# graehl/carmel

Hardware: AMD Instinct MI355X
Metric: arc-updates/sec (EM iterations/sec x derivation-lattice arcs swept per iteration) (higher is better)
Workload: dtype f64; 1 GPU; c4: synthetic 1000000-state / 9999990-arc WFST, 1000000 training pairs per GPU (random walks of 5-40 arcs), conditional normalisation, cached lattices; parallelism=corpus-sharded x1, none

## Files before the change

carmel_amd/csrc/engine.cpp:

```cpp
#include <hip/hip_runtime.h>
#include <chrono>
#include <cmath>
#include <cstdio>
#include <cstring>
#include <cstdlib>
#include <limits>
#include <string>
#include <thread>
#include <unordered_map>
#include <vector>
#include "engine.hpp"
#include "options.hpp"
#include "host/refhash.hpp"
#include "rng.hpp"
#include "unrolled_args.hpp"

int unrolled_try_build(carmel_hip_trainer* t, int host_threads, uint8_t* has_derivation, carmel_hip_lattice_stats* stats);
int gpu_build_lattices(carmel_hip_trainer* t, const BuildOptions& opt, uint8_t* has_derivation, carmel_hip_lattice_stats* stats,
                       bool& done);
int gpu_tables_for_host_layout(carmel_hip_trainer* t, const std::vector<uint32_t>& lane_arc, const std::vector<uint32_t>& wave_arc);
int carmel_hip_debug_lattice_fingerprint_impl(carmel_hip_trainer* t, uint64_t* out);
int build_run_tables(carmel_hip_trainer* t);
int exchange_weights_in(carmel_hip_trainer* t, ExchangePlan* xp, const TransArgs& T, bool need_x);
int exchange_counts_out(carmel_hip_trainer* t, ExchangePlan* xp, const TransArgs& T);
// ... 176 lines not shown
    int arc = weights_ahead_drop(t);
    if (arc) return arc;
  }
  layout_changed(t);
  if (t->scalars_pending) {
    (void)hipStreamSynchronize(t->side);
    t->scalars_pending = false;
  }
  t->build_prune = prune;
  t->build_threads = host_threads;
  if (t->matrix) {
    HIPCHK(hipStreamSynchronize(t->stream));
    matrix_release(t->matrix);
    t->matrix = nullptr;
  }
  {
    int rc = unrolled_try_build(t, host_threads, has_derivation, stats);
    if (rc) return rc;
    if (t->unrolled) return CARMEL_HIP_OK;
  }
  auto t0 = std::chrono::steady_clock::now();
  BuildOptions opt;
  opt.prune = prune != 0;
  opt.threads = host_threads;
  if (const char* e = lib_opt("lane_states")) opt.lane_states = (uint32_t)atoi(e);
  if (const char* e = lib_opt("tile_sweep")) opt.tile_sweep = atoi(e) != 0;
  if (const char* e = lib_opt("lane_fused")) opt.lane_fused = atoi(e) != 0;
  if (lib_opt("transpose") && atoi(lib_opt("transpose")) == 0) opt.lane_fused = false;
  if (const char* e = lib_opt("lane_chunks")) opt.lane_chunks = (uint32_t)std::max(1, atoi(e));
  if (const char* e = lib_opt("lane_window")) opt.lane_window = (uint32_t)std::max(0, atoi(e));
  if (const char* e = lib_opt("lane_window_min")) opt.lane_window_min = (uint32_t)std::max(0, atoi(e));
  if (const char* e = lib_opt("wave_ring")) opt.wave_ring = atoi(e) != 0;
  if (const char* e = lib_opt("wave_min_width")) opt.wave_min_width = opt.wave_lane_min_width = atof(e);
  {
    const bool want_gpu = !(lib_opt("gpu_build") && atoi(lib_opt("gpu_build")) == 0) &&
                          !(lib_opt("transpose") && atoi(lib_opt("transpose")) == 0);
    bool probe_ok = true;
    if (want_gpu && t->corpus.n_pairs > 4096) {
      const uint64_t np = t->corpus.n_pairs, n_probe = 64;
      for (uint64_t k = 0; k < n_probe && probe_ok; ++k) {
        const uint64_t p = k * (np / n_probe);
        PairLattice pl;
        bool hd = false;
        build_pair_lattice(t->w, t->corpus.in_sym.data() + t->corpus.in_off[p], (uint32_t)(t->corpus.in_off[p + 1] - t->corpus.in_off[p]),
                           t->corpus.out_sym.data() + t->corpus.out_off[p], (uint32_t)(t->corpus.out_off[p + 1] - t->corpus.out_off[p]),
                           opt.prune, pl, hd);
        if (pl.explored_states > 200 || (hd && (pl.n_states > opt.lane_states || pl.edges.size() > 200))) opt.gpu_large_caps = true;
        if (pl.explored_states > 1024 || (hd && (pl.cyclic || pl.n_states > 1023 || pl.edges.size() > 1536))) probe_ok = false;
      }
    }
    if (want_gpu && probe_ok) {
      bool done = false;
      int rc = gpu_build_lattices(t, opt, has_derivation, stats, done);
      if (rc) return rc;
      if (!done && !opt.gpu_large_caps) {
        opt.gpu_large_caps = true;
        rc = gpu_build_lattices(t, opt, has_derivation, stats, done);
        if (rc) return rc;
        if (!done) opt.gpu_large_caps = false;
      }
      if (done) {
        if (lib_opt("timing")) fprintf(stderr, "timing: lattices built on the GPU\n");
        rc = build_run_tables(t);
        if (stats) stats->device_bytes = t->device_bytes;
        return rc;
      }
// ... 1473 lines not shown
```

carmel_amd/csrc/host_api.cpp:

```cpp
#include <cstdlib>
#include <algorithm>
#include <cstring>
#include <string>
#include "../../include/carmel_hip.h"
#include "options.hpp"
#include "lattice.hpp"

using namespace carmel_hip;

struct carmel_hip_host_lattices {
  HostWfst w;
  HostCorpus c;
  LatticeSet L;
  std::string err;
};

extern "C" {

int carmel_hip_host_build(carmel_hip_host_lattices** out, uint32_t n_states, uint32_t final_state, uint64_t n_arcs,
                          const uint32_t* src, const uint32_t* dst, const uint32_t* in_sym, const uint32_t* out_sym,
                          uint64_t n_pairs, const uint64_t* in_off, const uint32_t* cin, const uint64_t* out_off,
                          const uint32_t* cout, const double* pair_weight, int prune, int threads,
                          uint32_t small_pairs, uint32_t small_states, int lane_states) {
  if (!out) return CARMEL_HIP_ERR_ARG;
  carmel_hip_host_lattices* h = new carmel_hip_host_lattices();
  h->w.n_states = n_states;
  h->w.final_state = final_state;
  h->w.n_arcs = n_arcs;
  h->w.src.assign(src, src + n_arcs);
  h->w.dst.assign(dst, dst + n_arcs);
  h->w.in.assign(in_sym, in_sym + n_arcs);
  h->w.out.assign(out_sym, out_sym + n_arcs);
  h->w.build_index();
  h->c.n_pairs = n_pairs;
  h->c.in_off.assign(in_off, in_off + n_pairs + 1);
  h->c.out_off.assign(out_off, out_off + n_pairs + 1);
  h->c.in_sym.assign(cin, cin + in_off[n_pairs]);
  h->c.out_sym.assign(cout, cout + out_off[n_pairs]);
  if (pair_weight)
    h->c.weight.assign(pair_weight, pair_weight + n_pairs);
  else
    h->c.weight.assign(n_pairs, 1.0);
  BuildOptions opt;
  opt.prune = prune != 0;
  opt.threads = threads;
  if (small_pairs) opt.small_pairs = small_pairs;
  if (small_states) opt.small_states = small_states;
  if (lane_states >= 0) opt.lane_states = (uint32_t)lane_states;
  if (const char* e = lib_opt("lane_window")) opt.lane_window = (uint32_t)std::max(0, atoi(e));
  if (const char* e = lib_opt("tile_sweep")) opt.tile_sweep = atoi(e) != 0;
  if (const char* e = lib_opt("lane_fused")) opt.lane_fused = atoi(e) != 0;
  if (const char* e = lib_opt("lane_window_min")) opt.lane_window_min = (uint32_t)std::max(0, atoi(e));
  if (lane_states == 0 && !lib_opt("wave_min_width")) opt.wave = false;
  if (const char* e = lib_opt("wave_ring")) opt.wave_ring = atoi(e) != 0;
  if (const char* e = lib_opt("wave_min_width")) opt.wave_min_width = opt.wave_lane_min_width = atof(e);
  if (!build_lattices(h->w, h->c, opt, h->L, h->err)) {
    delete h;
    return CARMEL_HIP_ERR_ARG;
  }
  *out = h;
  return CARMEL_HIP_OK;
}

void carmel_hip_host_dims(carmel_hip_host_lattices* h, uint64_t* dims) {
  dims[0] = h->L.bundles.size();
  dims[1] = h->L.in_off.size();
  dims[2] = h->L.in_arcs.size();
  dims[3] = h->L.level_off.size();
  dims[4] = h->L.pair_id.size();
  dims[5] = h->L.classes.size();
  dims[6] = h->L.n_kept;
  dims[7] = h->L.n_cyclic;
  dims[8] = h->L.explored_states;
  dims[9] = h->L.explored_arcs;
  dims[10] = h->L.lane_groups.size();
  dims[11] = h->L.lane_fwd.size();
  dims[12] = h->L.lane_pair.size();
  dims[13] = h->L.lane_classes.size();
  dims[14] = h->L.total_states;
  dims[15] = h->L.total_arcs;
  dims[16] = h->L.last_pre_states;
  dims[17] = h->L.last_post_states;
  dims[18] = h->L.last_post_arcs;
}

// ... 105 lines not shown
```

carmel_amd/csrc/lattice.cpp:

```cpp
#include "lattice.hpp"
#include "options.hpp"
#include <algorithm>
#include <functional>
#include <chrono>
#include <cmath>
#include <cstring>
#include <limits>
#include <numeric>
#include <thread>
#include <atomic>

namespace carmel_hip {
void build_transpose(LatticeSet& out, uint64_t n_arcs, int nt);


void HostWfst::build_index() {
  idx_off.assign((size_t)n_states + 1, 0);
  for (uint64_t k = 0; k < n_arcs; ++k) idx_off[src[k] + 1]++;
  for (uint32_t s = 0; s < n_states; ++s) idx_off[s + 1] += idx_off[s];
  idx_key.resize(n_arcs);
  idx_arc.resize(n_arcs);
  std::vector<uint64_t> cur(idx_off.begin(), idx_off.end() - 1);
  for (uint64_t k = 0; k < n_arcs; ++k) {
    uint64_t p = cur[src[k]]++;
// ... 504 lines not shown
                        bool prune, PairLattice& lat, bool& has_deriv) {
  Scratch sc;
  build_pair_lattice_impl(w, in, n_in, out, n_out, prune, lat, has_deriv, sc);
}

namespace {

struct BundlePlan {
  std::vector<uint32_t> pairs;
  uint64_t n_states = 0, n_arcs = 0;
  uint32_t n_levels = 0;
  bool cyclic = false;
};

}

bool build_lattices(const HostWfst& w, const HostCorpus& c, const BuildOptions& opt, LatticeSet& out,
                    std::string& err) {
  if (w.idx_off.size() != (size_t)w.n_states + 1) {
    err = "WFST index not built";
    return false;
  }
  const uint64_t np = c.n_pairs;
  const bool timing = lib_opt("timing") != nullptr;
  auto tick = std::chrono::steady_clock::now();
  auto phase = [&](const char* name) {
    if (!timing) return;
    auto now = std::chrono::steady_clock::now();
    fprintf(stderr, "timing: lattice build: %-28s %8.3f s\n", name, std::chrono::duration<double>(now - tick).count());
    tick = now;
  };
  std::vector<PairLattice> lats(np);
  out = LatticeSet();
  out.has_deriv.assign(np, 0);
  int nt = opt.threads > 0 ? opt.threads : std::min(32, (int)std::thread::hardware_concurrency());
  if (nt < 1) nt = 1;
  if ((uint64_t)nt > np) nt = (int)std::max<uint64_t>(1, np);
  {
    std::atomic<uint64_t> next(0);
    const uint64_t batch = std::max<uint64_t>(1, std::min<uint64_t>(256, np / ((uint64_t)nt * 8)));
    auto work = [&]() {
      Scratch sc;
      for (;;) {
        uint64_t p0 = next.fetch_add(batch);
        if (p0 >= np) break;
        uint64_t p1 = std::min(np, p0 + batch);
        for (uint64_t p = p0; p < p1; ++p) {
          bool hd = false;
          build_pair_lattice_impl(w, c.in_sym.data() + c.in_off[p], (uint32_t)(c.in_off[p + 1] - c.in_off[p]),
                                  c.out_sym.data() + c.out_off[p], (uint32_t)(c.out_off[p + 1] - c.out_off[p]),
                                  opt.prune, lats[p], hd, sc);
          out.has_deriv[p] = hd;
          PairLattice& L = lats[p];
          if (hd && !L.cyclic && opt.lane_window && L.n_states > opt.lane_window_min && L.n_states <= LANE_STATE_MASK) {
            std::vector<uint32_t>& cnt = sc.span_cnt;
            std::vector<uint32_t>& nid = sc.span_id;
            cnt.assign((size_t)L.n_levels + 2, 0);
            for (uint32_t st = 0; st < L.n_states; ++st) cnt[L.level[st] + 1]++;
            for (size_t k = 1; k < cnt.size(); ++k) cnt[k] += cnt[k - 1];
            nid.resize(L.n_states);
            for (uint32_t st = 0; st < L.n_states; ++st) nid[st] = cnt[L.level[st]]++;
            uint32_t sp = 1;
            for (auto& e : L.edges) sp = std::max(sp, nid[e.dst] - nid[e.src]);
            L.span = sp;
          }
        }
// ... 667 lines not shown
    for (uint64_t a = 0; a < w.n_arcs; ++a) cnt[a + 1] += cnt[a];
    const uint64_t total = cnt[w.n_arcs];
    out.arc_off = cnt;
    out.slot_pos.resize(total);
    in_threads([&](int t) {
      const uint64_t lo = arc_lo(t), hi = arc_lo(t + 1);
      for (uint64_t k = 0; k < nlane_rec; ++k) {
        const uint2_t r = out.lane_bwd[k];
        if ((r.x & LANE_VALID) && r.y >= lo && r.y < hi) out.slot_pos[cnt[r.y]++] = k;
      }
      for (uint64_t k = 0; k < nwave; ++k) {
        const uint32_t a = out.wave_bwd_arc[k];
        if (a != 0xffffffffu && a >= lo && a < hi) out.slot_pos[cnt[a]++] = out.wave_slot_base + k;
      }
      for (uint64_t k = 0; k < out.out_arcs.size(); ++k) {
        const uint32_t a = out.out_arcs[k].y;
        if (a >= lo && a < hi) out.slot_pos[cnt[a]++] = nlane + k;
      }
    });
    for (uint64_t a = 0; a < w.n_arcs; ++a)
      if (out.arc_off[a + 1] - out.arc_off[a] > 64)
        for (uint64_t j = out.arc_off[a]; j < out.arc_off[a + 1]; j += 4096) {
          out.hot_chunks.push_back(a);
          out.hot_chunks.push_back(j);
          out.hot_chunks.push_back(std::min(out.arc_off[a + 1], j + 4096));
        }
  }
  phase("slots by arc (counting sort)");
  build_transpose(out, w.n_arcs, nt);
  phase("transposition tables");
  return true;
}

void build_transpose(LatticeSet& out, uint64_t n_arcs, int nt) {
  const uint64_t N = out.slot_pos.size();
  out.t_buckets.clear();
  out.t_split_arcs.clear();
  if (N >= (1ull << 32) || N == 0) return;
  const uint64_t BK = out.bucket;
  {
    uint64_t a = 0;
    while (a < n_arcs) {
      uint64_t c = out.arc_off[a + 1] - out.arc_off[a];
      if (c > TRANS_HEAVY) {
        const bool split = c > BK;
        if (split) out.t_split_arcs.push_back((uint32_t)a);
        for (uint64_t g = out.arc_off[a]; g < out.arc_off[a + 1]; g += BK)
          out.t_buckets.push_back(TransBucket{g, (uint32_t)std::min<uint64_t>(BK, out.arc_off[a + 1] - g),
                                              (uint32_t)a, 1u, TRANS_SINGLE | (split ? TRANS_SPLIT : 0u)});
        ++a;
        continue;
      }
      uint64_t e = a, items = 0;
      while (e < n_arcs && e - a < BK) {
        uint64_t ce = out.arc_off[e + 1] - out.arc_off[e];
        if (ce > TRANS_HEAVY || items + ce > BK) break;
        items += ce;
        ++e;
      }
      out.t_buckets.push_back(TransBucket{out.arc_off[a], (uint32_t)items, (uint32_t)a, (uint32_t)(e - a), 0u});
      a = e;
    }
  }
  out.t_a_off.assign(n_arcs, 0);
  for (const TransBucket& B : out.t_buckets)
    if (!(B.flags & TRANS_SINGLE))
      for (uint32_t a = 0; a < B.n_arcs; ++a) out.t_a_off[B.arc_lo + a] = (uint16_t)(out.arc_off[B.arc_lo + a] - B.item_base);
  out.t_b_arc.assign(N, 0);
  out.t_b_rank.assign(N, 0);
  out.t_b_src.assign(N, 0);
  out.t_t_pos.assign(N, 0);
  out.t_t_src.assign(N, 0);
  const uint64_t tile_sz = out.tile;
  const uint64_t n_tiles = (out.n_post + tile_sz - 1) / tile_sz;
  out.t_tile_base.assign(n_tiles + 1, 0);
  std::vector<uint64_t> pos_of(N);
  {
    std::atomic<size_t> next(0);
    auto work = [&]() {
      std::vector<std::pair<uint64_t, uint32_t>> items;
      for (;;) {
        size_t b = next.fetch_add(16);
        if (b >= out.t_buckets.size()) break;
        size_t be = std::min(out.t_buckets.size(), b + 16);
        for (; b < be; ++b) {
          const TransBucket& B = out.t_buckets[b];
          items.resize(B.n_items);
          for (uint32_t r = 0; r < B.n_items; ++r) items[r] = {out.slot_pos[B.item_base + r], r};
          std::sort(items.begin(), items.end());
          uint64_t a = B.arc_lo;
          std::vector<uint16_t> arc_of_rank(B.n_items);
          if (B.flags & TRANS_SINGLE) {
            std::fill(arc_of_rank.begin(), arc_of_rank.end(), (uint16_t)0);
          } else {
// ... 57 lines not shown
```

carmel_amd/csrc/lattice.hpp:

```cpp
#pragma once
#include <cstdint>
#include <vector>
#include <string>

namespace carmel_hip {

struct HostWfst {
  uint32_t n_states = 0, final_state = 0;
  uint64_t n_arcs = 0;
  std::vector<uint32_t> src, dst, in, out, group;
  std::vector<uint64_t> idx_off;
  std::vector<uint64_t> idx_key;
  std::vector<uint32_t> idx_arc;
  void build_index();
};

struct HostCorpus {
  uint64_t n_pairs = 0;
  std::vector<uint64_t> in_off, out_off;
  std::vector<uint32_t> in_sym, out_sym;
  std::vector<double> weight;
};

struct PairLattice {
// ... 24 lines not shown
};
static_assert(sizeof(BundleDesc) == 64, "BundleDesc layout");

struct uint2_t {
  uint32_t x, y;
};

static const uint32_t LANE_CHUNK = 4;
static const uint32_t LANE_LAST = 0x80000000u;
static const uint32_t LANE_VALID = 0x40000000u;
static const uint32_t LANE_STATE_MASK = 0x3ffu;
static const uint32_t LANE_POS_SHIFT = 10;
static const uint32_t LANE_POS_MAX = (1u << 20) - 1;
#ifndef TRANS_K
#define TRANS_K 16
#endif
#ifndef TRANS_KT
#define TRANS_KT TRANS_K
#endif
#ifndef TRANS_KB
#define TRANS_KB TRANS_K
#endif
static const uint32_t TRANS_TILE = TRANS_KT * 1024, TRANS_BUCKET = TRANS_KB * 1024, TRANS_HEAVY = 2048, TRANS_SPLIT = 1u, TRANS_SINGLE = 2u;
static const uint32_t TILE_SWEEP_TILE = 8192, TILE_SWEEP_ALPHA_ROWS = 126, TILE_SWEEP_ROWS = 48, TILE_SWEEP_GROUPS = 16;
static const uint32_t TILE_SWEEP_LDS = TILE_SWEEP_TILE * 12 + TILE_SWEEP_ALPHA_ROWS * 64 * 8;
#ifndef LANE_FUSED_ROWS_N
#define LANE_FUSED_ROWS_N 16
#endif
static const uint32_t LANE_FUSED_ROWS = LANE_FUSED_ROWS_N, LANE_FUSED_TILE = LANE_FUSED_ROWS * 64;
struct TransBucket {
  uint64_t item_base;
  uint32_t n_items, arc_lo, n_arcs, flags;
};
struct LaneGroup {
  uint64_t stream_base;
  uint32_t maxlen;
  uint32_t n_lanes;
  uint32_t pair_base;
  uint32_t max_states;
  uint32_t window;
  uint32_t spill_row;
};
static_assert(sizeof(LaneGroup) == 32, "LaneGroup layout");

static const uint32_t WAVE_VALID = 0x80000000u;
static const uint32_t WAVE_MAX_STATES = 16384, WAVE_MAX_WIDTH = 1024;
static const uint32_t WAVE_RING_MAX = 1024, WAVE_RING_WIDTH = 64;
struct WaveDesc {
  uint64_t fwd_base;
  uint64_t bwd_base;
  uint32_t n_states, n_levels;
  uint32_t level_base;
  uint32_t pair;
  uint32_t max_width;
  uint32_t ring;
  double logw;
  uint64_t n_arcs;
  uint64_t spill_base;
};
static_assert(sizeof(WaveDesc) == 64, "WaveDesc layout");

struct LatticeSet {
  std::vector<WaveDesc> waves;
  std::vector<uint2_t> wave_fwd;
  std::vector<uint32_t> wave_bwd;
  std::vector<uint32_t> wave_bwd_arc;
// ... 9 lines not shown
  uint64_t wave_slot_base = 0;
  uint64_t wave_states = 0, wave_arcs = 0;
  std::vector<BundleDesc> bundles;
  std::vector<uint2_t> in_arcs, out_arcs;
  std::vector<uint32_t> in_off, out_off;
  std::vector<uint32_t> level_off;
  std::vector<uint32_t> pair_start, pair_final, pair_id;
  std::vector<double> pair_logw;
  struct LaunchClass {
    uint32_t first, count;
    uint32_t block;
    uint32_t max_states;
    bool serial;
  };
  std::vector<LaunchClass> classes;
  std::vector<LaneGroup> lane_groups;
  std::vector<uint2_t> lane_fwd, lane_bwd;
  std::vector<uint32_t> lane_pair, lane_nstates;
  std::vector<double> lane_logw;
  struct LaneClass {
    uint32_t first, count, max_states;
    uint32_t tile_first = 0, tile_count = 0;
    bool windowed = false;
  };
  uint64_t lane_spill_rows = 0;
  std::vector<LaneClass> lane_classes;
  bool lane_tiles_aligned = false;
  uint32_t tile = TRANS_TILE;
  bool tile_sweep = false;
  bool wave_gather = false;
  bool tables_deferred = false;
  bool lane_fused = false;
  uint32_t bucket = TRANS_BUCKET;
  std::vector<uint32_t> tile_group;
  uint64_t lane_states = 0, lane_arcs = 0;
  std::vector<uint32_t> state_orig;
  std::vector<uint64_t> arc_off;
  std::vector<uint64_t> slot_pos;
  std::vector<uint64_t> hot_chunks;
  uint64_t n_post = 0;
  std::vector<TransBucket> t_buckets;
  std::vector<uint64_t> t_tile_base;
  std::vector<uint16_t> t_b_arc;
  std::vector<uint16_t> t_b_rank;
  std::vector<uint32_t> t_b_src;
  std::vector<uint16_t> t_t_pos;
  std::vector<uint32_t> t_t_src;
  std::vector<uint16_t> t_a_off;
  std::vector<uint32_t> t_split_arcs;
  uint64_t total_states = 0, total_arcs = 0, max_levels = 0, n_cyclic = 0;
  uint64_t explored_states = 0, explored_arcs = 0;
  uint64_t last_pre_states = 0, last_post_states = 0, last_post_arcs = 0;
  std::vector<uint8_t> has_deriv;
  uint64_t n_kept = 0;
};

struct BuildOptions {
  bool prune = true;
  int threads = 0;
  uint32_t small_pairs = 64;
  uint32_t small_states = 2048;
  uint32_t lds_states_max = 16384;
  uint32_t lane_states = 96;
  uint32_t lane_window = 64;
  uint32_t lane_window_min = 40;
  bool keep_state_ids = false;
  bool gpu_large_caps = false;
  bool wave_ring = true;
  bool wave = true;
  double wave_min_width = 4.0;
  double wave_lane_min_width = 16.0;
  uint64_t wave_lane_threshold = 262144;
  uint32_t wave_lane_arcs = 2048;
  bool tile_sweep = true;
  bool wave_gather = false;
  bool device_tables = false;
  bool lane_fused = true;
  uint32_t lane_chunks = 1;
};

bool build_lattices(const HostWfst& w, const HostCorpus& c, const BuildOptions& opt, LatticeSet& out, std::string& err);

uint64_t assign_lane_classes(LatticeSet& out, const BuildOptions& opt, bool only_lanes);

void build_pair_lattice(const HostWfst& w, const uint32_t* in, uint32_t n_in, const uint32_t* out, uint32_t n_out,
                        bool prune, PairLattice& lat, bool& has_deriv);

}
```

carmel_amd/csrc/lattice_gpu.hip:

```cpp
#include <hip/hip_runtime.h>
#include <hipcub/hipcub.hpp>
#include <algorithm>
#include <chrono>
#include <functional>
#include <cmath>
#include <cstring>
#include <limits>
#include <vector>
#include "engine.hpp"
#include "options.hpp"

namespace {

struct GCaps {
  uint32_t cx, ce, ck, ch, threads;
};
const GCaps G_SMALL = {256, 448, 256, 512, 131072};
const GCaps G_LARGE = {1024, 2560, 1536, 2048, 65536};

enum { PF_HAS = 1, PF_FALLBACK = 2 };

struct GArgs {
  const uint64_t* idx_off;
  const uint64_t* idx_key;
// ... 507 lines not shown
  const uint32_t* rb = rec_bwd + (size_t)p * GK;
  const uint32_t* ra = rec_arc + (size_t)p * GK;
  for (uint32_t k = 0; k < e; ++k) {
    const uint32_t x = rf[k];
    const uint32_t bp = ((x >> LANE_POS_SHIFT) & LANE_POS_MAX) + shift;
    f[(size_t)k * 64] = (x & ~(LANE_POS_MAX << LANE_POS_SHIFT)) | (bp << LANE_POS_SHIFT);
    b[(size_t)(shift + k) * 64] = rb[k];
    items[it + k] = ((unsigned long long)ra[k] << 32) | (unsigned long long)(g.stream_base + (uint64_t)(shift + k) * 64 + lane);
  }
}

__global__ void slots_kernel(const unsigned long long* items, uint64_t n, uint64_t n_arcs, uint64_t* slot_pos, uint64_t* arc_off) {
  const uint64_t i = (uint64_t)blockIdx.x * blockDim.x + threadIdx.x;
  if (i >= n) return;
  const uint32_t a = (uint32_t)(items[i] >> 32);
  slot_pos[i] = items[i] & 0xffffffffull;
  const uint32_t prev = i ? (uint32_t)(items[i - 1] >> 32) : 0u;
  for (uint64_t x = (i ? (uint64_t)prev + 1 : 0); x <= a; ++x) arc_off[x] = i;
  if (i + 1 == n)
    for (uint64_t x = (uint64_t)a + 1; x <= n_arcs; ++x) arc_off[x] = n;
}

__global__ void bucket_end_kernel(const uint64_t* arc_off, uint64_t n_arcs, uint32_t* b_end, uint32_t BK ) {
  const uint64_t a = (uint64_t)blockIdx.x * blockDim.x + threadIdx.x;
  if (a >= n_arcs) return;
  const uint64_t limit = arc_off[a] + BK;
  uint64_t lo = a, hi = min(n_arcs, a + (uint64_t)BK);
  while (lo < hi) {
    const uint64_t m = (lo + hi + 1) >> 1;
    if (arc_off[m] <= limit) lo = m; else hi = m - 1;
  }
  b_end[a] = (uint32_t)lo;
}
__global__ void heavy_list_kernel(const uint64_t* arc_off, uint64_t n_arcs, uint32_t* list, uint32_t cap, uint32_t* n) {
  const uint64_t a = (uint64_t)blockIdx.x * blockDim.x + threadIdx.x;
  if (a >= n_arcs || arc_off[a + 1] - arc_off[a] <= TRANS_HEAVY) return;
  const uint32_t k = atomicAdd(n, 1u);
  if (k < cap) list[k] = (uint32_t)a;
}
__global__ void bucket_chain_kernel(const uint64_t* arc_off, const uint32_t* b_end, uint64_t n_arcs, const uint32_t* heavy,
                                    uint32_t n_heavy, TransBucket* buckets, uint32_t* split_arcs, uint32_t cap,
                                    uint32_t* n_out , uint32_t BK ) {
  if (blockIdx.x || threadIdx.x) return;
  uint64_t a = 0;
  uint32_t nb = 0, ns = 0, hp = 0;
  bool over = false;
  while (a < n_arcs) {
    const uint64_t c = arc_off[a + 1] - arc_off[a];
    if (c > TRANS_HEAVY) {
      const bool split = c > BK;
      if (split) {
        if (ns < cap) split_arcs[ns] = (uint32_t)a;
        ++ns;
      }
      for (uint64_t g = arc_off[a]; g < arc_off[a + 1]; g += BK) {
        if (nb < cap)
          buckets[nb] = TransBucket{g, (uint32_t)min((uint64_t)BK, arc_off[a + 1] - g), (uint32_t)a, 1u,
                                    TRANS_SINGLE | (split ? TRANS_SPLIT : 0u)};
        else
          over = true;
        ++nb;
      }
      ++a;
      continue;
    }
    uint64_t e = b_end[a];
    while (hp < n_heavy && heavy[hp] < a) ++hp;
    if (hp < n_heavy && heavy[hp] < e) e = heavy[hp];
    if (e == a) e = a + 1;
    if (nb < cap)
      buckets[nb] = TransBucket{arc_off[a], (uint32_t)(arc_off[e] - arc_off[a]), (uint32_t)a, (uint32_t)(e - a), 0u};
// ... 295 lines not shown
  fp(3, t->lane_pair.p, t->lane_pair.bytes());
  fp(4, t->lane_nstates.p, t->lane_nstates.bytes());
  fp(5, t->lane_logw.p, t->lane_logw.bytes());
  fp(6, t->t_buckets.p, t->t_buckets.bytes());
  fp(7, t->t_tile_base.p, t->t_tile_base.bytes());
  fp(8, t->t_b_arc.p, t->t_b_arc.bytes() & ~(size_t)3);
  fp(9, t->t_b_rank.p, t->t_b_rank.bytes() & ~(size_t)3);
  fp(10, t->t_b_src.p, t->t_b_src.bytes());
  fp(11, t->t_t_pos.p, t->t_t_pos.bytes() & ~(size_t)3);
  fp(12, t->t_t_src.p, t->t_t_src.bytes());
  fp(13, t->t_a_off.p, t->t_a_off.bytes() & ~(size_t)3);
  fp(14, t->t_split_arcs.p, t->t_split_arcs.bytes());
  fp(15, t->pair_w.p, t->pair_w.bytes());
  HIPCHK(hipGetLastError());
  HIPCHK(hipMemcpyAsync(out, acc.p, 16 * 8, hipMemcpyDeviceToHost, s));
  HIPCHK(hipStreamSynchronize(s));
  return CARMEL_HIP_OK;
}

static int gpu_tables_from_items(carmel_hip_trainer* t, DevBuf<char>& tmp, DevBuf<unsigned long long>& items, DevBuf<unsigned long long>& items_sorted,
                                 uint64_t n_items, uint64_t n_sort, uint64_t n_post, const std::function<void(const char*)>& lap) {
  const HostWfst& w = t->w;
  const LatticeSet& L = t->lat;
  hipStream_t s = t->stream;
  HIPCHK(sort_keys(tmp, items.p, items_sorted.p, n_sort, 32 + bits_for(w.n_arcs + 1), s));
  HIPCHK(t->arc_off.alloc(w.n_arcs + 1));
  HIPCHK(t->slot_pos.alloc(n_items));
  hipLaunchKernelGGL(slots_kernel, dim3((unsigned)((n_items + 255) / 256)), dim3(256), 0, s, items_sorted.p, n_items, w.n_arcs,
                     t->slot_pos.p, t->arc_off.p);
  t->hot_chunks.release();
  lap("slots by arc");
  DevBuf<uint32_t> b_end, d_nout;
  HIPCHK(b_end.alloc(w.n_arcs));
  HIPCHK(d_nout.alloc(4));
  hipLaunchKernelGGL(bucket_end_kernel, dim3((unsigned)((w.n_arcs + 255) / 256)), dim3(256), 0, s, t->arc_off.p, w.n_arcs, b_end.p, L.bucket);
  const uint32_t cap = (uint32_t)(2 * (n_items / L.bucket) + w.n_arcs / L.bucket + 2 * (n_items / TRANS_HEAVY) + 16);
  HIPCHK(t->t_buckets.alloc(cap));
  HIPCHK(t->t_split_arcs.alloc(cap));
  DevBuf<uint32_t> heavy, heavy_sorted;
  HIPCHK(heavy.alloc(cap));
  HIPCHK(heavy_sorted.alloc(cap));
  HIPCHK(hipMemsetAsync(d_nout.p, 0, 16, s));
  hipLaunchKernelGGL(heavy_list_kernel, dim3((unsigned)((w.n_arcs + 255) / 256)), dim3(256), 0, s, t->arc_off.p, w.n_arcs, heavy.p, cap,
                     d_nout.p + 3);
  uint32_t n_heavy = 0;
  HIPCHK(hipMemcpyAsync(&n_heavy, d_nout.p + 3, 4, hipMemcpyDeviceToHost, s));
  HIPCHK(hipStreamSynchronize(s));
  if (n_heavy > cap) return fail(CARMEL_HIP_ERR_HIP, "gpu lattice build: heavy-arc list overflow");
  if (n_heavy) HIPCHK(sort_keys(tmp, heavy.p, heavy_sorted.p, n_heavy, 32, s));
  hipLaunchKernelGGL(bucket_chain_kernel, dim3(1), dim3(1), 0, s, t->arc_off.p, b_end.p, w.n_arcs, heavy_sorted.p, n_heavy,
                     t->t_buckets.p, t->t_split_arcs.p, cap, d_nout.p, L.bucket);
  uint32_t h_nout[4] = {0, 0, 0, 0};
  HIPCHK(hipMemcpyAsync(h_nout, d_nout.p, 12, hipMemcpyDeviceToHost, s));
  HIPCHK(hipStreamSynchronize(s));
  if (h_nout[2]) return fail(CARMEL_HIP_ERR_HIP, "gpu lattice build: bucket table overflow");
  const uint32_t n_buckets = h_nout[0], n_split = h_nout[1];
  t->t_buckets.n = n_buckets;
  t->t_split_arcs.n = n_split;
  lap("buckets");
  const uint64_t n_tiles = (n_post + L.tile - 1) / L.tile;
  HIPCHK(t->t_a_off.alloc(w.n_arcs));
  HIPCHK(hipMemsetAsync(t->t_a_off.p, 0, w.n_arcs * 2, s));
  hipLaunchKernelGGL(a_off_kernel, dim3(n_buckets), dim3(256), 0, s, t->t_buckets.p, n_buckets, t->arc_off.p, t->t_a_off.p);
  DevBuf<unsigned long long> bkey, bkey_sorted;
  DevBuf<uint32_t> bval, bval_sorted, tile_key, tile_sorted, Jv, J_sorted;
  HIPCHK(bkey.alloc(n_items));
  HIPCHK(bkey_sorted.alloc(n_items));
  HIPCHK(bval.alloc(n_items));
  HIPCHK(bval_sorted.alloc(n_items));
  hipLaunchKernelGGL(bucket_key_kernel, dim3((unsigned)((n_items + 255) / 256)), dim3(256), 0, s, t->t_buckets.p, n_buckets,
                     t->slot_pos.p, n_items, bkey.p, bval.p);
  HIPCHK(sort_pairs(tmp, bkey.p, bkey_sorted.p, bval.p, bval_sorted.p, n_items, 32 + bits_for(n_buckets), s));
  HIPCHK(t->t_b_arc.alloc(n_items));
  HIPCHK(t->t_b_rank.alloc(n_items));
  HIPCHK(t->t_b_src.alloc(n_items));
  HIPCHK(t->t_t_pos.alloc(n_items));
  HIPCHK(t->t_t_src.alloc(n_items));
  HIPCHK(t->t_tile_base.alloc(n_tiles + 1));
  HIPCHK(tile_key.alloc(n_items));
  HIPCHK(tile_sorted.alloc(n_items));
  HIPCHK(Jv.alloc(n_items));
  HIPCHK(J_sorted.alloc(n_items));
  hipLaunchKernelGGL(bucket_major_kernel, dim3((unsigned)((n_items + 255) / 256)), dim3(256), 0, s, t->t_buckets.p, bkey_sorted.p,
                     bval_sorted.p, items_sorted.p, n_items, L.tile, t->t_b_arc.p, t->t_b_rank.p, tile_key.p, Jv.p);
  HIPCHK(sort_pairs(tmp, tile_key.p, tile_sorted.p, Jv.p, J_sorted.p, n_items, bits_for(n_tiles), s));
  hipLaunchKernelGGL(tile_major_kernel, dim3((unsigned)((n_items + 255) / 256)), dim3(256), 0, s, tile_sorted.p, J_sorted.p,
                     bkey_sorted.p, n_items, n_tiles, L.tile, t->t_t_src.p, t->t_t_pos.p, t->t_b_src.p, t->t_tile_base.p);
  HIPCHK(hipGetLastError());
  HIPCHK(t->t_x.alloc(n_items));
// ... 175 lines not shown
    hipLaunchKernelGGL(classify_kernel, dim3(1024), dim3(256), 0, s, CA, pp_win.p, d_stats.p);
    HIPCHK(hipMemcpyAsync(hc, d_stats.p, 32, hipMemcpyDeviceToHost, s));
    HIPCHK(hipStreamSynchronize(s));
  }
  const uint64_t n_plain = hc[0], n_win = hc[1];
  if (hc[2]) return CARMEL_HIP_OK;
  if (opt.wave && hc[3] && n_plain + n_win < opt.wave_lane_threshold) return CARMEL_HIP_OK;
  DevBuf<unsigned long long> key, key_sorted;
  DevBuf<char> tmp;
  HIPCHK(key.alloc(np));
  HIPCHK(key_sorted.alloc(np));
  hipLaunchKernelGGL(pair_key_kernel, dim3((unsigned)((np + 255) / 256)), dim3(256), 0, s, pp_E.p, pp_S.p, pp_flags.p, pp_win.p, np, key.p);
  HIPCHK(sort_keys(tmp, key.p, key_sorted.p, np, 64, s));
  const size_t ng_plain = (size_t)((n_plain + 63) / 64), ng = ng_plain + (size_t)((n_win + 63) / 64);
  SlotMap SM;
  SM.n_plain = n_plain;
  SM.n_win = n_win;
  SM.ng_plain = (uint32_t)ng_plain;
  DevBuf<uint32_t> g_maxlen, g_maxstates, g_items, g_window;
  HIPCHK(g_maxlen.alloc(ng));
  HIPCHK(g_maxstates.alloc(ng));
  HIPCHK(g_items.alloc(ng));
  HIPCHK(g_window.alloc(ng));
  hipLaunchKernelGGL(group_dims_kernel, dim3((unsigned)ng), dim3(64), 0, s, key_sorted.p, pp_E.p, pp_S.p, pp_win.p, SM, g_maxlen.p,
                     g_maxstates.p, g_items.p, g_window.p);
  std::vector<uint32_t> h_maxlen(ng), h_maxstates(ng), h_items(ng), h_window(ng);
  HIPCHK(hipMemcpyAsync(h_maxlen.data(), g_maxlen.p, ng * 4, hipMemcpyDeviceToHost, s));
  HIPCHK(hipMemcpyAsync(h_maxstates.data(), g_maxstates.p, ng * 4, hipMemcpyDeviceToHost, s));
  HIPCHK(hipMemcpyAsync(h_items.data(), g_items.p, ng * 4, hipMemcpyDeviceToHost, s));
  HIPCHK(hipMemcpyAsync(h_window.data(), g_window.p, ng * 4, hipMemcpyDeviceToHost, s));
  HIPCHK(hipStreamSynchronize(s));
  LatticeSet& L = t->lat;
  L = LatticeSet();
  L.lane_groups.resize(ng);
  std::vector<unsigned long long> h_item_off(ng);
  uint64_t spill_rows = 0;
  {
    unsigned long long acc = 0;
    for (size_t g = 0; g < ng; ++g) {
      LaneGroup& Gd = L.lane_groups[g];
      std::memset(&Gd, 0, sizeof Gd);
      Gd.n_lanes = (uint32_t)(g < ng_plain ? std::min<uint64_t>(64, n_plain - g * 64) : std::min<uint64_t>(64, n_win - (g - ng_plain) * 64));
      Gd.pair_base = (uint32_t)(g * 64);
      Gd.maxlen = h_maxlen[g];
      const uint32_t win = g < ng_plain ? 0u : h_window[g];
      Gd.max_states = win ? win : h_maxstates[g];
      Gd.window = win;
      if (win) {
        if (spill_rows + h_maxstates[g] > 0xffffffffull) return CARMEL_HIP_OK;
        Gd.spill_row = (uint32_t)spill_rows;
        spill_rows += h_maxstates[g];
      }
      h_item_off[g] = acc;
      acc += h_items[g];
    }
  }
  L.lane_spill_rows = spill_rows;
  const uint64_t n_rec = assign_lane_classes(L, opt, true);
  if (n_rec >= (1ull << 32)) return CARMEL_HIP_OK;
  lap("pair sort + lane groups");
  HIPCHK(t->lane_groups.upload(L.lane_groups, s));
  if (L.tile_sweep)
    HIPCHK(t->tile_group.upload(L.tile_group, s));
  else
    t->tile_group.release();
  DevBuf<unsigned long long> d_item_off, items, items_sorted;
// ... 145 lines not shown
```

carmel_amd/csrc/options.cpp:

```cpp
#include "options.hpp"
#include <cstdlib>
#include <cstring>
#include <mutex>
#include <string>
#include "../../include/carmel_hip.h"

namespace carmel_hip {
namespace {
const char* const kKeys[] = {
    "timing",
    "lane_states", "tile_sweep", "lane_fused", "transpose", "lane_chunks", "lane_window", "lane_window_min", "wave_ring", "wave_min_width",
    "gpu_build", "wave_gather", "wave_xc", "tile_gather", "device_tables", "trans_scatter", "trans_runs", "lane_fused_kernel",
    "tile_sweep_kernel", "mailbox", "poison", "lane_trace", "exchange_sparse", "mstep_wide", "trans_bucket_walk",
    "weights_ahead",
    "dense", "unrolled", "unrolled_ragged",
    "gibbs_chains", "gibbs_own_cap", "gibbs_workgroup", "gibbs_clk", "gibbs_reg", "gibbs_lane", "forest_sweep", "forest_ldswalk", "forest_multi",
    "forest_nohash", "forest_trace", "forest_exact_host", "forest_exact_clk", "forest_logdomain", "forest_gcol", "forest_gather",
    "decode_lds", "decode_chunk_bytes"};
constexpr int kN = (int)(sizeof kKeys / sizeof kKeys[0]);
const char* volatile g_val[kN];
std::mutex g_mu;
int find(const char* key) {
  for (int i = 0; i < kN; ++i)
    if (!std::strcmp(kKeys[i], key)) return i;
  return -1;
}
}
const char* lib_opt(const char* key) {
  const int i = find(key);
  return i < 0 ? nullptr : g_val[i];
}
bool lib_opt_off(const char* key) {
  const char* v = lib_opt(key);
  return v && std::atoi(v) == 0;
}
}

extern "C" {
int carmel_hip_set_option(const char* key, const char* value) {
  using namespace carmel_hip;
  if (!key) return CARMEL_HIP_ERR_ARG;
  const int i = find(key);
  if (i < 0) return CARMEL_HIP_ERR_ARG;
  std::lock_guard<std::mutex> lk(g_mu);
  if (!value)
    g_val[i] = nullptr;
  else {
    char* c = (char*)std::malloc(std::strlen(value) + 1);
    if (!c) return CARMEL_HIP_ERR_HIP;
    std::strcpy(c, value);
    g_val[i] = c;
  }
  return CARMEL_HIP_OK;
}
const char* carmel_hip_get_option(const char* key) { return key ? carmel_hip::lib_opt(key) : nullptr; }
int carmel_hip_option_count(void) { return carmel_hip::kN; }
const char* carmel_hip_option_name(int i) { return i >= 0 && i < carmel_hip::kN ? carmel_hip::kKeys[i] : nullptr; }
}
```

carmel_amd/csrc/options.hpp:

```cpp
#pragma once
namespace carmel_hip {
const char* lib_opt(const char* key);
inline bool lib_opt_set(const char* key) { return lib_opt(key) != nullptr; }
bool lib_opt_off(const char* key);
}
```

Before: 57.56 billion arc-updates/s.

## Balance transposition buckets into equal shares across device compute units

Replaces greedy transposition bucket chaining with a planner that sizes light-arc buckets so the total bucket count fills whole rounds of CU-multiple slots. Heavy arcs keep their fixed-size split buckets. A binary search picks the smallest share that fits the round budget, and a GPU kernel cuts the buckets. The aim is to remove tail imbalance in the per-iteration transpose/scatter pass. In exchange, build time goes up, and fewer, larger light buckets may reduce locality.

Result: no change. 57.02 billion arc-updates/s (median of 2 runs) (-0.9%).

```diff
diff --git a/carmel_amd/csrc/engine.cpp b/carmel_amd/csrc/engine.cpp
--- a/carmel_amd/csrc/engine.cpp
+++ b/carmel_amd/csrc/engine.cpp
@@ -232,6 +232,11 @@
   if (const char* e = lib_opt("lane_window_min")) opt.lane_window_min = (uint32_t)std::max(0, atoi(e));
   if (const char* e = lib_opt("wave_ring")) opt.wave_ring = atoi(e) != 0;
   if (const char* e = lib_opt("wave_min_width")) opt.wave_min_width = opt.wave_lane_min_width = atof(e);
+  {
+    hipDeviceProp_t prop;
+    HIPCHK(hipGetDeviceProperties(&prop, t->device));
+    opt.bucket_slots = bucket_slots_opt(prop.multiProcessorCount > 8 ? (unsigned)prop.multiProcessorCount / 8 * 8 : 8u);
+  }
   {
     const bool want_gpu = !(lib_opt("gpu_build") && atoi(lib_opt("gpu_build")) == 0) &&
                           !(lib_opt("transpose") && atoi(lib_opt("transpose")) == 0);
diff --git a/carmel_amd/csrc/host_api.cpp b/carmel_amd/csrc/host_api.cpp
--- a/carmel_amd/csrc/host_api.cpp
+++ b/carmel_amd/csrc/host_api.cpp
@@ -51,6 +51,7 @@
   if (const char* e = lib_opt("tile_sweep")) opt.tile_sweep = atoi(e) != 0;
   if (const char* e = lib_opt("lane_fused")) opt.lane_fused = atoi(e) != 0;
   if (const char* e = lib_opt("lane_window_min")) opt.lane_window_min = (uint32_t)std::max(0, atoi(e));
+  opt.bucket_slots = bucket_slots_opt(0);
   if (lane_states == 0 && !lib_opt("wave_min_width")) opt.wave = false;
   if (const char* e = lib_opt("wave_ring")) opt.wave_ring = atoi(e) != 0;
   if (const char* e = lib_opt("wave_min_width")) opt.wave_min_width = opt.wave_lane_min_width = atof(e);
diff --git a/carmel_amd/csrc/lattice.cpp b/carmel_amd/csrc/lattice.cpp
--- a/carmel_amd/csrc/lattice.cpp
+++ b/carmel_amd/csrc/lattice.cpp
@@ -560,6 +560,7 @@
   };
   std::vector<PairLattice> lats(np);
   out = LatticeSet();
+  out.bucket_slots = opt.bucket_slots;
   out.has_deriv.assign(np, 0);
   int nt = opt.threads > 0 ? opt.threads : std::min(32, (int)std::thread::hardware_concurrency());
   if (nt < 1) nt = 1;
@@ -1293,6 +1294,41 @@
   return true;
 }
 
+bool plan_balanced_buckets(std::vector<BucketGroup>& groups, uint64_t max_light, uint32_t cap, uint32_t slots, uint32_t extra_rounds,
+                           BucketPlan& plan) {
+  plan = BucketPlan();
+  if (!slots || max_light >= cap) return false;
+  uint64_t heavy = 0;
+  for (const BucketGroup& G : groups)
+    if (bucket_group_heavy(G)) heavy += (G.n_items + cap - 1) / cap;
+  const auto light_of = [](const BucketGroup& G, uint64_t g) { return std::max<uint64_t>(1, (G.n_items + g - 1) / g); };
+  const auto count = [&](uint64_t g) {
+    uint64_t n = heavy;
+    for (const BucketGroup& G : groups)
+      if (!bucket_group_heavy(G)) n += light_of(G, g);
+    return n;
+  };
+  const uint64_t g_max = cap - max_light;
+  const uint64_t rounds = std::max<uint64_t>(1, (count(g_max) + slots - 1) / slots) + extra_rounds, room = rounds * slots;
+  if (room >= (1ull << 31)) return false;
+  uint64_t lo = 1, hi = g_max;
+  while (lo < hi) {
+    const uint64_t mid = (lo + hi) >> 1;
+    if (count(mid) <= room) hi = mid; else lo = mid + 1;
+  }
+  uint32_t first = 0;
+  for (BucketGroup& G : groups) {
+    G.n_buckets = (uint32_t)(bucket_group_heavy(G) ? (G.n_items + cap - 1) / cap : light_of(G, lo));
+    G.bucket_first = first;
+    first += G.n_buckets;
+  }
+  plan.rounds = (uint32_t)rounds;
+  plan.share = (uint32_t)lo;
+  plan.heavy_buckets = (uint32_t)heavy;
+  plan.n_buckets = first;
+  return true;
+}
+
 void build_transpose(LatticeSet& out, uint64_t n_arcs, int nt) {
   const uint64_t N = out.slot_pos.size();
   out.t_buckets.clear();
@@ -1321,6 +1357,32 @@
       }
       out.t_buckets.push_back(TransBucket{out.arc_off[a], (uint32_t)items, (uint32_t)a, (uint32_t)(e - a), 0u});
       a = e;
+    }
+  }
+  out.bucket_plan = BucketPlan();
+  if (out.bucket_slots && BK == TRANS_BUCKET && out.t_buckets.size() > out.bucket_slots) {
+    std::vector<BucketGroup> groups;
+    uint64_t max_light = 0;
+    const auto items_of = [&](uint64_t a) { return out.arc_off[a + 1] - out.arc_off[a]; };
+    for (uint64_t a = 0; a < n_arcs;) {
+      uint64_t e = a + 1;
+      if (items_of(a) <= TRANS_HEAVY) {
+        while (e < n_arcs && items_of(e) <= TRANS_HEAVY) ++e;
+        for (uint64_t x = a; x < e; ++x) max_light = std::max(max_light, items_of(x));
+      }
+      groups.push_back(BucketGroup{a, e, out.arc_off[a], out.arc_off[e] - out.arc_off[a], 0u, 0u});
+      a = e;
+    }
+    BucketPlan plan;
+    if (plan_balanced_buckets(groups, max_light, (uint32_t)BK, out.bucket_slots, TRANS_BALANCE_EXTRA_ROUNDS, plan)) {
+      std::vector<TransBucket> cut(plan.n_buckets);
+      bool ok = true;
+      for (const BucketGroup& G : groups)
+        for (uint32_t k = 0; k < G.n_buckets; ++k) ok = balanced_bucket(out.arc_off.data(), G, k, (uint32_t)BK, cut[G.bucket_first + k]) && ok;
+      if (ok) {
+        out.t_buckets.swap(cut);
+        out.bucket_plan = plan;
+      }
     }
   }
   out.t_a_off.assign(n_arcs, 0);
diff --git a/carmel_amd/csrc/lattice.hpp b/carmel_amd/csrc/lattice.hpp
--- a/carmel_amd/csrc/lattice.hpp
+++ b/carmel_amd/csrc/lattice.hpp
@@ -80,6 +80,46 @@
   uint64_t item_base;
   uint32_t n_items, arc_lo, n_arcs, flags;
 };
+#ifndef TRANS_BALANCE_EXTRA_ROUNDS
+#define TRANS_BALANCE_EXTRA_ROUNDS 0
+#endif
+struct BucketGroup {
+  uint64_t arc_lo, arc_hi;
+  uint64_t item_lo, n_items;
+  uint32_t n_buckets, bucket_first;
+};
+struct BucketPlan {
+  uint32_t rounds = 0, share = 0, heavy_buckets = 0, n_buckets = 0;
+};
+bool plan_balanced_buckets(std::vector<BucketGroup>& groups, uint64_t max_light, uint32_t cap, uint32_t slots, uint32_t extra_rounds,
+                           BucketPlan& plan);
+static inline bool bucket_group_heavy(const BucketGroup& G) { return G.arc_hi == G.arc_lo + 1 && G.n_items > TRANS_HEAVY; }
+#if defined(__HIPCC__)
+#define CARMEL_HOST_DEVICE __host__ __device__
+#else
+#define CARMEL_HOST_DEVICE
+#endif
+CARMEL_HOST_DEVICE inline uint64_t balanced_bucket_end(const uint64_t* arc_off, const BucketGroup& G, uint32_t k) {
+  if (k + 1 >= G.n_buckets) return G.arc_hi;
+  const uint64_t limit = G.item_lo + (uint64_t)(k + 1) * G.n_items / G.n_buckets;
+  uint64_t lo = G.arc_lo, hi = G.arc_hi;
+  while (lo < hi) {
+    const uint64_t mid = (lo + hi + 1) >> 1;
+    if (arc_off[mid] <= limit) lo = mid; else hi = mid - 1;
+  }
+  return lo;
+}
+CARMEL_HOST_DEVICE inline bool balanced_bucket(const uint64_t* arc_off, const BucketGroup& G, uint32_t k, uint32_t cap, TransBucket& B) {
+  if (G.arc_hi == G.arc_lo + 1 && G.n_items > TRANS_HEAVY) {
+    const uint64_t g = G.item_lo + (uint64_t)k * cap, left = G.item_lo + G.n_items - g;
+    B = TransBucket{g, (uint32_t)(left < cap ? left : cap), (uint32_t)G.arc_lo, 1u, TRANS_SINGLE | (G.n_items > cap ? TRANS_SPLIT : 0u)};
+    return true;
+  }
+  const uint64_t a = k ? balanced_bucket_end(arc_off, G, k - 1) : G.arc_lo, e = balanced_bucket_end(arc_off, G, k);
+  const uint64_t items = arc_off[e] - arc_off[a];
+  B = TransBucket{arc_off[a], (uint32_t)items, (uint32_t)a, (uint32_t)(e - a), 0u};
+  return items <= cap && e - a <= cap && e > a && (items > 0 || G.n_items == 0);
+}
 struct LaneGroup {
   uint64_t stream_base;
   uint32_t maxlen;
@@ -155,6 +195,8 @@
   bool tables_deferred = false;
   bool lane_fused = false;
   uint32_t bucket = TRANS_BUCKET;
+  uint32_t bucket_slots = 0;
+  BucketPlan bucket_plan;
   std::vector<uint32_t> tile_group;
   uint64_t lane_states = 0, lane_arcs = 0;
   std::vector<uint32_t> state_orig;
@@ -199,6 +241,7 @@
   bool wave_gather = false;
   bool device_tables = false;
   bool lane_fused = true;
+  uint32_t bucket_slots = 0;
   uint32_t lane_chunks = 1;
 };
 
diff --git a/carmel_amd/csrc/lattice_gpu.hip b/carmel_amd/csrc/lattice_gpu.hip
--- a/carmel_amd/csrc/lattice_gpu.hip
+++ b/carmel_amd/csrc/lattice_gpu.hip
@@ -563,11 +563,39 @@
   }
   b_end[a] = (uint32_t)lo;
 }
-__global__ void heavy_list_kernel(const uint64_t* arc_off, uint64_t n_arcs, uint32_t* list, uint32_t cap, uint32_t* n) {
+__global__ void heavy_list_kernel(const uint64_t* arc_off, uint64_t n_arcs, uint32_t* list, uint32_t cap, uint32_t* n, uint32_t* max_light) {
   const uint64_t a = (uint64_t)blockIdx.x * blockDim.x + threadIdx.x;
-  if (a >= n_arcs || arc_off[a + 1] - arc_off[a] <= TRANS_HEAVY) return;
-  const uint32_t k = atomicAdd(n, 1u);
-  if (k < cap) list[k] = (uint32_t)a;
+  uint32_t light = 0;
+  if (a < n_arcs) {
+    const uint64_t c = arc_off[a + 1] - arc_off[a];
+    if (c > TRANS_HEAVY) {
+      const uint32_t k = atomicAdd(n, 1u);
+      if (k < cap) list[k] = (uint32_t)a;
+    } else
+      light = (uint32_t)c;
+  }
+  for (int o = 32; o > 0; o >>= 1) light = max(light, (uint32_t)__shfl_down(light, o, 64));
+  if ((threadIdx.x & 63) == 0 && light) atomicMax(max_light, light);
+}
+__global__ void heavy_off_kernel(const uint64_t* arc_off, const uint32_t* heavy, uint32_t n_heavy, uint64_t* off) {
+  const uint32_t k = blockIdx.x * blockDim.x + threadIdx.x;
+  if (k >= n_heavy) return;
+  off[2 * k] = arc_off[heavy[k]];
+  off[2 * k + 1] = arc_off[heavy[k] + 1];
+}
+__global__ void balanced_bucket_kernel(const uint64_t* arc_off, const BucketGroup* groups, uint32_t n_groups, uint32_t n_buckets, uint32_t BK,
+                                       TransBucket* buckets, uint32_t* bad) {
+  const uint32_t b = blockIdx.x * blockDim.x + threadIdx.x;
+  if (b >= n_buckets) return;
+  uint32_t lo = 0, hi = n_groups - 1;
+  while (lo < hi) {
+    const uint32_t m = (lo + hi + 1) >> 1;
+    if (groups[m].bucket_first <= b) lo = m; else hi = m - 1;
+  }
+  const BucketGroup G = groups[lo];
+  TransBucket B;
+  if (!balanced_bucket(arc_off, G, b - G.bucket_first, BK, B)) atomicOr(bad, 1u);
+  buckets[b] = B;
 }
 __global__ void bucket_chain_kernel(const uint64_t* arc_off, const uint32_t* b_end, uint64_t n_arcs, const uint32_t* heavy,
                                     uint32_t n_heavy, TransBucket* buckets, uint32_t* split_arcs, uint32_t cap,
@@ -929,7 +957,7 @@
   lap("slots by arc");
   DevBuf<uint32_t> b_end, d_nout;
   HIPCHK(b_end.alloc(w.n_arcs));
-  HIPCHK(d_nout.alloc(4));
+  HIPCHK(d_nout.alloc(8));
   hipLaunchKernelGGL(bucket_end_kernel, dim3((unsigned)((w.n_arcs + 255) / 256)), dim3(256), 0, s, t->arc_off.p, w.n_arcs, b_end.p, L.bucket);
   const uint32_t cap = (uint32_t)(2 * (n_items / L.bucket) + w.n_arcs / L.bucket + 2 * (n_items / TRANS_HEAVY) + 16);
   HIPCHK(t->t_buckets.alloc(cap));
@@ -937,21 +965,92 @@
   DevBuf<uint32_t> heavy, heavy_sorted;
   HIPCHK(heavy.alloc(cap));
   HIPCHK(heavy_sorted.alloc(cap));
-  HIPCHK(hipMemsetAsync(d_nout.p, 0, 16, s));
+  HIPCHK(hipMemsetAsync(d_nout.p, 0, 32, s));
   hipLaunchKernelGGL(heavy_list_kernel, dim3((unsigned)((w.n_arcs + 255) / 256)), dim3(256), 0, s, t->arc_off.p, w.n_arcs, heavy.p, cap,
-                     d_nout.p + 3);
-  uint32_t n_heavy = 0;
-  HIPCHK(hipMemcpyAsync(&n_heavy, d_nout.p + 3, 4, hipMemcpyDeviceToHost, s));
+                     d_nout.p + 3, d_nout.p + 4);
+  uint32_t h_heavy[2] = {0, 0};
+  HIPCHK(hipMemcpyAsync(h_heavy, d_nout.p + 3, 8, hipMemcpyDeviceToHost, s));
   HIPCHK(hipStreamSynchronize(s));
+  const uint32_t n_heavy = h_heavy[0];
   if (n_heavy > cap) return fail(CARMEL_HIP_ERR_HIP, "gpu lattice build: heavy-arc list overflow");
   if (n_heavy) HIPCHK(sort_keys(tmp, heavy.p, heavy_sorted.p, n_heavy, 32, s));
-  hipLaunchKernelGGL(bucket_chain_kernel, dim3(1), dim3(1), 0, s, t->arc_off.p, b_end.p, w.n_arcs, heavy_sorted.p, n_heavy,
-                     t->t_buckets.p, t->t_split_arcs.p, cap, d_nout.p, L.bucket);
-  uint32_t h_nout[4] = {0, 0, 0, 0};
-  HIPCHK(hipMemcpyAsync(h_nout, d_nout.p, 12, hipMemcpyDeviceToHost, s));
-  HIPCHK(hipStreamSynchronize(s));
-  if (h_nout[2]) return fail(CARMEL_HIP_ERR_HIP, "gpu lattice build: bucket table overflow");
-  const uint32_t n_buckets = h_nout[0], n_split = h_nout[1];
+  uint32_t n_buckets = 0, n_split = 0;
+  bool have_greedy = false;
+  auto greedy = [&]() -> int {
+    hipLaunchKernelGGL(bucket_chain_kernel, dim3(1), dim3(1), 0, s, t->arc_off.p, b_end.p, w.n_arcs, heavy_sorted.p, n_heavy,
+                       t->t_buckets.p, t->t_split_arcs.p, cap, d_nout.p, L.bucket);
+    uint32_t h_nout[4] = {0, 0, 0, 0};
+    HIPCHK(hipMemcpyAsync(h_nout, d_nout.p, 12, hipMemcpyDeviceToHost, s));
+    HIPCHK(hipStreamSynchronize(s));
+    if (h_nout[2]) return fail(CARMEL_HIP_ERR_HIP, "gpu lattice build: bucket table overflow");
+    n_buckets = h_nout[0];
+    n_split = h_nout[1];
+    have_greedy = true;
+    return CARMEL_HIP_OK;
+  };
+  t->lat.bucket_plan = BucketPlan();
+  bool balanced = false;
+  if (L.bucket_slots && L.bucket == TRANS_BUCKET) {
+    if ((n_items + L.bucket - 1) / L.bucket <= L.bucket_slots) {
+      int rc = greedy();
+      if (rc) return rc;
+    }
+    if (!have_greedy || n_buckets > L.bucket_slots) {
+      std::vector<uint32_t> h_arc(n_heavy);
+      std::vector<uint64_t> h_off(2 * (size_t)n_heavy);
+      if (n_heavy) {
+        DevBuf<uint64_t> d_off;
+        HIPCHK(d_off.alloc(2 * (size_t)n_heavy));
+        hipLaunchKernelGGL(heavy_off_kernel, dim3((n_heavy + 255) / 256), dim3(256), 0, s, t->arc_off.p, heavy_sorted.p, n_heavy, d_off.p);
+        HIPCHK(hipMemcpyAsync(h_arc.data(), heavy_sorted.p, (size_t)n_heavy * 4, hipMemcpyDeviceToHost, s));
+        HIPCHK(hipMemcpyAsync(h_off.data(), d_off.p, (size_t)n_heavy * 16, hipMemcpyDeviceToHost, s));
+        HIPCHK(hipStreamSynchronize(s));
+      }
+      std::vector<BucketGroup> groups;
+      std::vector<uint32_t> split;
+      uint64_t arc = 0, item = 0;
+      for (uint32_t k = 0; k <= n_heavy; ++k) {
+        const uint64_t a = k < n_heavy ? h_arc[k] : w.n_arcs, i0 = k < n_heavy ? h_off[2 * k] : n_items;
+        if (a > arc) groups.push_back(BucketGroup{arc, a, item, i0 - item, 0u, 0u});
+        if (k == n_heavy) break;
+        groups.push_back(BucketGroup{a, a + 1, i0, h_off[2 * k + 1] - i0, 0u, 0u});
+        if (h_off[2 * k + 1] - i0 > L.bucket) split.push_back((uint32_t)a);
+        arc = a + 1;
+        item = h_off[2 * k + 1];
+      }
+      BucketPlan plan;
+      if (plan_balanced_buckets(groups, h_heavy[1], L.bucket, L.bucket_slots, TRANS_BALANCE_EXTRA_ROUNDS, plan)) {
+        DevBuf<BucketGroup> d_groups;
+        DevBuf<TransBucket> cut;
+        HIPCHK(d_groups.upload(groups, s));
+        HIPCHK(cut.alloc(plan.n_buckets));
+        hipLaunchKernelGGL(balanced_bucket_kernel, dim3((plan.n_buckets + 255) / 256), dim3(256), 0, s, t->arc_off.p, d_groups.p,
+                           (uint32_t)groups.size(), plan.n_buckets, L.bucket, cut.p, d_nout.p + 5);
+        uint32_t bad = 1;
+        HIPCHK(hipMemcpyAsync(&bad, d_nout.p + 5, 4, hipMemcpyDeviceToHost, s));
+        HIPCHK(hipStreamSynchronize(s));
+        if (!bad) {
+          std::swap(t->t_buckets.p, cut.p);
+          std::swap(t->t_buckets.n, cut.n);
+          if (!split.empty())
+            HIPCHK(hipMemcpyAsync(t->t_split_arcs.p, split.data(), split.size() * 4, hipMemcpyHostToDevice, s));
+          HIPCHK(hipStreamSynchronize(s));
+          n_buckets = plan.n_buckets;
+          n_split = (uint32_t)split.size();
+          t->lat.bucket_plan = plan;
+          balanced = true;
+        }
+      }
+    }
+  }
+  if (!balanced && !have_greedy) {
+    int rc = greedy();
+    if (rc) return rc;
+  }
+  if (lib_opt("timing"))
+    fprintf(stderr, "timing: transposition buckets: %u (%s: %u rounds of %u slots, share %u, %u heavy buckets)\n", n_buckets,
+            balanced ? "equal shares" : "greedy", t->lat.bucket_plan.rounds, L.bucket_slots, t->lat.bucket_plan.share,
+            t->lat.bucket_plan.heavy_buckets);
   t->t_buckets.n = n_buckets;
   t->t_split_arcs.n = n_split;
   lap("buckets");
@@ -1193,6 +1292,7 @@
   HIPCHK(hipStreamSynchronize(s));
   LatticeSet& L = t->lat;
   L = LatticeSet();
+  L.bucket_slots = opt.bucket_slots;
   L.lane_groups.resize(ng);
   std::vector<unsigned long long> h_item_off(ng);
   uint64_t spill_rows = 0;
diff --git a/carmel_amd/csrc/options.cpp b/carmel_amd/csrc/options.cpp
--- a/carmel_amd/csrc/options.cpp
+++ b/carmel_amd/csrc/options.cpp
@@ -12,7 +12,7 @@
     "lane_states", "tile_sweep", "lane_fused", "transpose", "lane_chunks", "lane_window", "lane_window_min", "wave_ring", "wave_min_width",
     "gpu_build", "wave_gather", "wave_xc", "tile_gather", "device_tables", "trans_scatter", "trans_runs", "lane_fused_kernel",
     "tile_sweep_kernel", "mailbox", "poison", "lane_trace", "exchange_sparse", "mstep_wide", "trans_bucket_walk",
-    "weights_ahead",
+    "weights_ahead", "trans_bucket_balance", "trans_bucket_slots",
     "dense", "unrolled", "unrolled_ragged",
     "gibbs_chains", "gibbs_own_cap", "gibbs_workgroup", "gibbs_clk", "gibbs_reg", "gibbs_lane", "forest_sweep", "forest_ldswalk", "forest_multi",
     "forest_nohash", "forest_trace", "forest_exact_host", "forest_exact_clk", "forest_logdomain", "forest_gcol", "forest_gather",
@@ -33,6 +33,13 @@
 bool lib_opt_off(const char* key) {
   const char* v = lib_opt(key);
   return v && std::atoi(v) == 0;
+}
+unsigned bucket_slots_opt(unsigned device_slots) {
+  if (lib_opt_off("trans_bucket_balance")) return 0;
+  const char* v = lib_opt("trans_bucket_slots");
+  if (!v) return device_slots;
+  const long n = std::atol(v);
+  return n <= 0 ? 0u : (unsigned)((n > (1l << 20) ? (1l << 20) : n) + 7) / 8 * 8;
 }
 }
 
diff --git a/carmel_amd/csrc/options.hpp b/carmel_amd/csrc/options.hpp
--- a/carmel_amd/csrc/options.hpp
+++ b/carmel_amd/csrc/options.hpp
@@ -3,4 +3,5 @@
 const char* lib_opt(const char* key);
 inline bool lib_opt_set(const char* key) { return lib_opt(key) != nullptr; }
 bool lib_opt_off(const char* key);
+unsigned bucket_slots_opt(unsigned device_slots);
 }
```
